# r-barnes/richdem

Measured on NVIDIA H100. Metric: Priority-Flood fill + D8 flow accumulation throughput, higher is better.
Workload: dtype f32

## Files before the change

richdem_b200/csrc/accum.cu:

```cuda
#include "flowmet.cuh"

#include <cmath>
#include <cooperative_groups.h>
namespace cg = cooperative_groups;

namespace rdb {

namespace {

constexpr uint32_t kDepsMask = 0xFFu;
constexpr uint32_t kSrcFlag = 0x80000000u;
constexpr int kCodeSole = 32;
constexpr int kCodeSource = 64;
constexpr int kLaneChunk = 1024;

template <bool DINF>
__global__ void __launch_bounds__(256) flow_code_kernel(const float *__restrict__ dem, uint8_t *__restrict__ code,
                                                         float *__restrict__ rmaxArr, double *__restrict__ accum,
                                                         int W, int H, float nodata, int ones, int tfilter) {
  const size_t n = (size_t)W * H;
  const size_t i = (size_t)blockIdx.x * blockDim.x + threadIdx.x;
  if (i >= n) return;
  const int y = (int)(i / W), x = (int)(i - (size_t)y * W);
  int cd;
// ... 1292 lines not shown
                      DinfShare *share, unsigned long long *stats, int ghost_lo_end, int ghost_hi_start, int seeded) {
  Ctx &c = ctx();
  int per_sm = 0;
  if (stats) RDB_CK(cudaOccupancyMaxActiveBlocksPerMultiprocessor(&per_sm, accum_walk_dinf_lanes_kernel<true>, 256, 0));
  else RDB_CK(cudaOccupancyMaxActiveBlocksPerMultiprocessor(&per_sm, accum_walk_dinf_lanes_kernel<false>, 256, 0));
  if (per_sm < 1) per_sm = 1;
  long long nb = (long long)c.num_sms * per_sm;
  const long long work = seeded >= 0 ? ((long long)seeded + 31) / 32 : ((long long)ncells + kLaneChunk - 1) / kLaneChunk;
  if (nb * 8 > work) nb = (work + 7) / 8;
  if (seeded >= 0 && nb < c.num_sms) nb = c.num_sms;
  if (nb < 1) nb = 1;
  if (seeded >= 0) {
    dinf_share_seed_kernel<<<1, 1, 0, c.stream>>>(share, seeded, (int)nb * 8, ncells);
    RDB_CK(cudaGetLastError());
  }
  const uint8_t *a_code = code;
  const float *a_rmax = rmax;
  int a_w = W, a_n = ncells;
  int *a_list = list;
  unsigned a_cap = (unsigned)ncells;
  DinfShare *a_sh = share;
  int a_excess = (int)(c.params.accum_dinf_share >= 0 ? c.params.accum_dinf_share : 1);
  int a_wait = (int)(c.params.accum_dinf_wait > 0 ? c.params.accum_dinf_wait : 4);
  if (a_excess > kLaneQueueD - 96) a_excess = kLaneQueueD - 96;
  unsigned long long *a_stats = stats;
  int a_lo = ghost_lo_end, a_hi = ghost_hi_start, a_seeded = seeded >= 0 ? 1 : 0;
  void *args[] = {(void *)&a_code, (void *)&a_rmax, (void *)&word, (void *)&a_w, (void *)&a_n, (void *)&a_list, (void *)&a_cap,
                  (void *)&a_sh, (void *)&a_excess, (void *)&a_wait, (void *)&a_stats, (void *)&a_lo, (void *)&a_hi, (void *)&a_seeded};
  if (stats)
    RDB_CK(cudaLaunchCooperativeKernel((const void *)accum_walk_dinf_lanes_kernel<true>, dim3((unsigned)nb), dim3(256), args, 0, c.stream));
  else
    RDB_CK(cudaLaunchCooperativeKernel((const void *)accum_walk_dinf_lanes_kernel<false>, dim3((unsigned)nb), dim3(256), args, 0, c.stream));
  RDB_CK(cudaGetLastError());
}

template <bool BAND>
void launch_walk_packed(const uint8_t *code, unsigned long long *word, int W, int ncells, const int *frontier,
                        int ghost_lo_end, int ghost_hi_start, bool src_in_code, int *cursor_buf = nullptr) {
  Ctx &c = ctx();
  if (ncells <= 0) return;
  if (c.params.accum_walk_lanes) {
    DevBuf<int> cursor;
    if (!cursor_buf) cursor.alloc(1);
    int *cur = cursor_buf ? cursor_buf : cursor.p;
    RDB_CK(cudaMemsetAsync(cur, 0, sizeof(int), c.stream));
    int per_sm = 0;
    RDB_CK(cudaOccupancyMaxActiveBlocksPerMultiprocessor(&per_sm, accum_walk_packed_lanes_kernel<BAND>, 256, 0));
    if (per_sm < 1) per_sm = 1;
    long long blocks = (long long)c.num_sms * per_sm;
    const long long need = ((long long)ncells + kLaneChunk - 1) / kLaneChunk;
    if (blocks * 8 > need) blocks = (need + 7) / 8;
    const int in_code = src_in_code && c.params.accum_walk_scan && (ncells & 3) == 0 && ((uintptr_t)code & 3) == 0 ? (int)c.params.accum_walk_scan : 0;
    int ahead = (int)(c.params.accum_walk_ahead > 0 ? c.params.accum_walk_ahead : 64);
    if (ahead > kLaneQueue - 128) ahead = kLaneQueue - 128;
    if (ahead < 32) ahead = 32;
    accum_walk_packed_lanes_kernel<BAND><<<(unsigned)blocks, 256, 0, c.stream>>>(code, word, W, ncells, frontier, ghost_lo_end,
                                                                               ghost_hi_start, cur, in_code, ahead);
    RDB_CK(cudaGetLastError());
    if (!cursor_buf) RDB_CK(cudaStreamSynchronize(c.stream));
  } else {
    accum_walk_packed_kernel<BAND><<<(unsigned)((ncells + 255) / 256), 256, 0, c.stream>>>(code, word, W, ncells, frontier,
                                                                                        ghost_lo_end, ghost_hi_start);
  }
}

__global__ void __launch_bounds__(256) band_take_packed_kernel(unsigned long long *ghost, double *sum, int *cnt, int W,
                                                                int *total) {
  const int x = blockIdx.x * blockDim.x + threadIdx.x;
  int k = 0;
  if (x < W) {
    const unsigned long long wv = ghost[x];
    k = (int)(wv >> 56);
    sum[x] = (double)(wv & kPkVal);
    cnt[x] = k;
    ghost[x] = 0;
  }
  for (int o = 16; o > 0; o >>= 1) k += __shfl_down_sync(0xffffffffu, k, o);
  if ((threadIdx.x & 31) == 0 && k) atomicAdd(total, k);
}

__global__ void __launch_bounds__(256) band_count_packed_kernel(const unsigned long long *__restrict__ gtop,
                                                                 const unsigned long long *__restrict__ gbot, int W,
                                                                 int *sums) {
  int s0 = 0, s1 = 0;
  for (int x = blockIdx.x * blockDim.x + threadIdx.x; x < W; x += gridDim.x * blockDim.x) {
    if (gtop) s0 += (int)(gtop[x] >> 56);
    if (gbot) s1 += (int)(gbot[x] >> 56);
  }
  for (int o = 16; o > 0; o >>= 1) {
    s0 += __shfl_down_sync(0xffffffffu, s0, o);
    s1 += __shfl_down_sync(0xffffffffu, s1, o);
  }
  if ((threadIdx.x & 31) == 0) {
    if (s0) atomicAdd(&sums[0], s0);
    if (s1) atomicAdd(&sums[1], s1);
  }
}

__global__ void __launch_bounds__(256) band_apply_packed_kernel(unsigned long long *row, const double *__restrict__ sum,
                                                                 const int *__restrict__ cnt, int W, int base_index,
                                                                 int *frontier, int *fcount, double scale) {
  const int x = blockIdx.x * blockDim.x + threadIdx.x;
  if (x >= W) return;
  const int k = cnt[x];
  if (k <= 0) return;
  const unsigned long long wv = row[x];
  const unsigned long long val = (wv & kPkVal) + (unsigned long long)sum[x];
  const unsigned long long left = (wv >> 56) - (unsigned long long)k;
  if (left == 0) {
    row[x] = (unsigned long long)__double_as_longlong((double)val * scale);
    frontier[atomicAdd(fcount, 1)] = base_index + x;
  } else {
    row[x] = (left << 56) | val;
  }
}

constexpr int kFaT = 64;
constexpr int kFaCells = kFaT * kFaT;
constexpr int kFaSlots = 4 * kFaT;
constexpr unsigned long long kLkOne = 1ull << 32;

__device__ __forceinline__ int fa_side(int left) { return left < kFaT ? left : kFaT; }

__device__ __forceinline__ int fa_slot_of(int lx, int ly, int tw, int th) {
  if (ly == 0) return lx;
  if (ly == th - 1) return kFaT + lx;
  if (lx == 0) return 2 * kFaT + ly;
  if (lx == tw - 1) return 3 * kFaT + ly;
  return -1;
}

__device__ __forceinline__ bool fa_slot_cell(int s, int tw, int th, int &lx, int &ly) {
  const int k = s & (kFaT - 1), side = s / kFaT;
  if (side < 2) {
    lx = k;
    ly = side == 0 ? 0 : th - 1;
    return k < tw && (side == 0 || th > 1);
  }
  lx = side == 2 ? 0 : tw - 1;
  ly = k;
  return k > 0 && k < th - 1 && (side == 2 || tw > 1);
}

constexpr int kFaRootExit = 0x8000, kFaRootEnd = 0x4000, kFaRoot = kFaRootExit | kFaRootEnd;

__device__ __forceinline__ int fa_tile_parent(int c, int cd, int tw, int th) {
  const int d = cd & 15;
  if (cd == kCodeNoData || d == 0) return c | kFaRootEnd;
  const int x = (c & (kFaT - 1)) + d8dx(d), y = c / kFaT + d8dy(d);
  if (x < 0 || y < 0 || x >= tw || y >= th) return c | kFaRootExit;
  return y * kFaT + x;
}

template <bool SUM>
__device__ __forceinline__ void fa_tile_jump(uint16_t *sPar, unsigned *sAcc, unsigned live) {
  constexpr int kPer = kFaCells / 256;
  const int t = threadIdx.x;
  while (__syncthreads_or(live)) {
    unsigned pq[kPer], a[kPer];
#pragma unroll
    for (int k = 0; k < kPer; k++) {
      if (live >> k & 1) {
        const int c = t + 256 * k, p = sPar[c], q = sPar[p];
        if (SUM) {
          pq[k] = (unsigned)p | (unsigned)q << 16;
          a[k] = sAcc[c];
        } else {
          sPar[c] = (uint16_t)q;
          if (q & kFaRoot) live &= ~(1u << k);
        }
      }
    }
    if (SUM) {
      __syncthreads();
#pragma unroll
      for (int k = 0; k < kPer; k++) {
        if (live >> k & 1) {
          const int q = pq[k] >> 16;
          atomicAdd(&sAcc[pq[k] & 0xffffu], a[k]);
          sPar[t + 256 * k] = (uint16_t)q;
          if (q & kFaRoot) live &= ~(1u << k);
        }
      }
    }
  }
}

__global__ void __launch_bounds__(256) fa_tile_codes_kernel(const float *__restrict__ dem, uint8_t *__restrict__ code,
                                                             int *__restrict__ link, unsigned long long *__restrict__ lword,
                                                             unsigned *__restrict__ inflow, int W, int H, float nodata,
                                                             int tiles_x) {
  constexpr int kWin = kFaT + 2;
  static_assert(kFaCells * sizeof(uint16_t) <= kWin * kWin * sizeof(float), "the parent array lives in the DEM window");
  __shared__ __align__(16) float sDem[kWin * kWin];
  __shared__ __align__(16) uint8_t sCode[kFaCells];
  __shared__ unsigned sCount[kFaSlots];
  const int t = threadIdx.x, tile = blockIdx.x;
  sCount[t] = 0;
  const int bx = tile % tiles_x, by = tile / tiles_x;
  const int x0 = bx * kFaT, y0 = by * kFaT;
  const int tw = fa_side(W - x0), th = fa_side(H - y0);
  constexpr unsigned kFaNoDataBits = 0x7fffffffu;
  for (int i = t; i < kWin * kWin; i += 256) {
    const int wy = i / kWin, wx = i - wy * kWin;
    const int gy = y0 - 1 + wy, gx = x0 - 1 + wx;
    float v = __uint_as_float(kFaNoDataBits);
    if (gy >= 0 && gy < H && gx >= 0 && gx < W) {
      v = __ldg(dem + (size_t)gy * W + gx);
      v = v == nodata ? __uint_as_float(kFaNoDataBits) : v != v ? __uint_as_float(0x7fc00000u) : v;
    }
    sDem[i] = v;
  }
  __syncthreads();
  {
    const int lx0 = (t & 15) * 4, ly0 = (t >> 4) * 4;
    float a[3][6];
#pragma unroll
    for (int j = 1; j < 3; j++)
#pragma unroll
      for (int k = 0; k < 6; k++) a[j][k] = sDem[(ly0 + j - 1) * kWin + lx0 + k];
#pragma unroll
    for (int j = 0; j < 4; j++) {
      const int ly = ly0 + j, gy = y0 + ly;
#pragma unroll
      for (int k = 0; k < 6; k++) {
        a[0][k] = a[1][k];
        a[1][k] = a[2][k];
        a[2][k] = sDem[(ly + 2) * kWin + lx0 + k];
      }
      unsigned word = 0;
#pragma unroll
      for (int k = 0; k < 4; k++) {
        const int lx = lx0 + k, gx = x0 + lx;
        const float e = a[1][k + 1];
        int cd = 0;
        if (lx >= tw || ly >= th || __float_as_uint(e) == kFaNoDataBits) {
          cd = kCodeNoData;
        } else if (!(gx == 0 || gy == 0 || gx == W - 1 || gy == H - 1)) {
          const float ne[9] = {0.f, a[1][k], a[0][k], a[0][k + 1], a[0][k + 2], a[1][k + 2], a[2][k + 2], a[2][k + 1], a[2][k]};
          float lowest = fminf(e, 3.402823466e+38f);
#pragma unroll
          for (int n = 1; n <= 8; n++) {
            if (ne[n] < lowest) {
              lowest = ne[n];
              cd = n;
            }
          }
        }
        word |= (unsigned)cd << (8 * k);
      }
      *reinterpret_cast<unsigned *>(&sCode[ly * kFaT + lx0]) = word;
    }
  }
  __syncthreads();
  reinterpret_cast<uint4 *>(code + (size_t)tile * kFaCells)[t] = reinterpret_cast<const uint4 *>(sCode)[t];
  uint16_t *sPar = reinterpret_cast<uint16_t *>(sDem);
  unsigned live = 0;
#pragma unroll
  for (int k = 0; k < kFaCells / 256; k++) {
    const int c = t + 256 * k, p = fa_tile_parent(c, sCode[c], tw, th);
    sPar[c] = (uint16_t)p;
    if (!(p & kFaRoot)) live |= 1u << k;
  }
  fa_tile_jump<false>(sPar, nullptr, live);
#pragma unroll
  for (int k = 0; k < kFaCells / 256; k++) {
    const int r = sPar[t + 256 * k];
    if (r & kFaRootExit) atomicAdd(&sCount[fa_slot_of(r & (kFaT - 1), (r & (kFaCells - 1)) / kFaT, tw, th)], 1u);
  }
  __syncthreads();
  const size_t gs = (size_t)tile * kFaSlots + t;
  int lk = -1;
  unsigned long long out = 0;
  int lx, ly;
  if (fa_slot_cell(t, tw, th, lx, ly)) {
    const int c = ly * kFaT + lx, r = sPar[c];
    if (r == (c | kFaRootExit)) {
      const int d = sCode[c] & 15;
      const int gx = x0 + lx + d8dx(d), gy = y0 + ly + d8dy(d), rbx = gx / kFaT, rby = gy / kFaT;
      const int rs = fa_slot_of(gx - rbx * kFaT, gy - rby * kFaT, fa_side(W - rbx * kFaT), fa_side(H - rby * kFaT));
      lk = -2 - ((rby * tiles_x + rbx) * kFaSlots + rs);
      out = kLkOne | sCount[t];
    } else if (r & kFaRootExit) {
      const int e = r & (kFaCells - 1);
      lk = tile * kFaSlots + fa_slot_of(e & (kFaT - 1), e / kFaT, tw, th);
    }
  }
  link[gs] = lk;
  lword[gs] = out;
  inflow[gs] = 0;
}

__device__ __forceinline__ int fa_link_next(const int *link, int r) {
  const int l = link[r];
  return l <= -2 ? r : l;
}

__global__ void __launch_bounds__(256) fa_link_count_kernel(const int *__restrict__ link, unsigned long long *lword,
                                                             int nslots) {
  const int p = blockIdx.x * blockDim.x + threadIdx.x;
  if (p >= nslots) return;
  const int l = link[p];
  if (l > -2) return;
  const int q = fa_link_next(link, -2 - l);
  if (q >= 0) atomicAdd(&lword[q], kLkOne);
}

__global__ void __launch_bounds__(256) fa_link_walk_kernel(const int *__restrict__ link, unsigned long long *lword,
                                                            unsigned *inflow, int nslots) {
  const int p = blockIdx.x * blockDim.x + threadIdx.x;
  if (p >= nslots) return;
  int l = link[p];
  if (l > -2) return;
  const unsigned long long old = atomicAdd(&lword[p], 0ull - kLkOne);
  if ((old >> 32) != 1ull) return;
  unsigned long long acc = old & (kLkOne - 1);
  for (;;) {
    const int r = -2 - l;
    atomicAdd(&inflow[r], (unsigned)acc);
    const int q = fa_link_next(link, r);
    if (q < 0) break;
    const unsigned long long o = atomicAdd(&lword[q], acc - kLkOne);
    if ((o >> 32) != 1ull) break;
    acc = (o & (kLkOne - 1)) + acc;
    l = link[q];
  }
}

__global__ void __launch_bounds__(256) fa_tile_final_kernel(const uint8_t *__restrict__ code,
                                                             const unsigned *__restrict__ inflow, double *__restrict__ accum,
                                                             int W, int H, int tiles_x) {
  constexpr unsigned kNoDataAcc = 0xffffffffu;
  __shared__ __align__(16) unsigned sAcc[kFaCells];
  __shared__ __align__(16) uint16_t sPar[kFaCells];
  __shared__ __align__(16) uint8_t sCode[kFaCells];
  const int t = threadIdx.x, tile = blockIdx.x;
  const int bx = tile % tiles_x, by = tile / tiles_x;
  const int x0 = bx * kFaT, y0 = by * kFaT;
  const int tw = fa_side(W - x0), th = fa_side(H - y0);
  reinterpret_cast<uint4 *>(sCode)[t] = __ldg(reinterpret_cast<const uint4 *>(code + (size_t)tile * kFaCells) + t);
  __syncthreads();
  unsigned live = 0;
#pragma unroll
  for (int k = 0; k < kFaCells / 256; k++) {
    const int c = t + 256 * k, cd = sCode[c], p = fa_tile_parent(c, cd, tw, th);
    sPar[c] = (uint16_t)p;
    sAcc[c] = cd == kCodeNoData ? kNoDataAcc : 1u;
    if (!(p & kFaRoot)) live |= 1u << k;
  }
  __syncthreads();
  int lx, ly;
  if (fa_slot_cell(t, tw, th, lx, ly) && sCode[ly * kFaT + lx] != kCodeNoData)
    sAcc[ly * kFaT + lx] += __ldg(inflow + (size_t)tile * kFaSlots + t);
  fa_tile_jump<true>(sPar, sAcc, live);
  for (int c = 2 * t; c < kFaCells; c += 512) {
    const int cx = c & (kFaT - 1), cy = c / kFaT;
    if (cx >= tw || cy >= th) continue;
    const unsigned s0 = sAcc[c], s1 = sAcc[c + 1];
    const double a0 = s0 == kNoDataAcc ? -1.0 : (double)s0, a1 = s1 == kNoDataAcc ? -1.0 : (double)s1;
    double *out = accum + (size_t)(y0 + cy) * W + x0 + cx;
    if (cx + 1 < tw && ((uintptr_t)out & 15) == 0) {
      *reinterpret_cast<double2 *>(out) = make_double2(a0, a1);
    } else {
      out[0] = a0;
      if (cx + 1 < tw) out[1] = a1;
    }
  }
}

long long fa_tile_slots(int w, int h) {
  return (long long)((w + kFaT - 1) / kFaT) * ((h + kFaT - 1) / kFaT) * kFaSlots;
}

void fa_d8_tiles(const float *d_dem, double *d_accum, int w, int h, float nodata) {
  Ctx &c = ctx();
  const int tiles_x = (w + kFaT - 1) / kFaT;
  const long long nslots = fa_tile_slots(w, h);
  const unsigned ntiles = (unsigned)(nslots / kFaSlots);
  DevBuf<uint8_t> code((size_t)ntiles * kFaCells);
  DevBuf<int> link((size_t)nslots);
  DevBuf<unsigned long long> lword((size_t)nslots);
  DevBuf<unsigned> inflow((size_t)nslots);
  const unsigned sblocks = (unsigned)((nslots + 255) / 256);
  fa_tile_codes_kernel<<<ntiles, 256, 0, c.stream>>>(d_dem, code.p, link.p, lword.p, inflow.p, w, h, nodata, tiles_x);
  fa_link_count_kernel<<<sblocks, 256, 0, c.stream>>>(link.p, lword.p, (int)nslots);
  KernelTimer kt;
  fa_link_walk_kernel<<<sblocks, 256, 0, c.stream>>>(link.p, lword.p, inflow.p, (int)nslots);
  kt.stop_async();
  fa_tile_final_kernel<<<ntiles, 256, 0, c.stream>>>(code.p, inflow.p, d_accum, w, h, tiles_x);
  RDB_CK(cudaGetLastError());
  count_launch(4);
  RDB_CK(cudaStreamSynchronize(c.stream));
  c.stats.ms_main_kernel += kt.ms();
  c.stats.accum_rounds = 1;
}
}

void fa_fused_dev(const float *d_dem, double *d_accum, int w, int h, float nodata, bool ones, bool dinf) {
  Ctx &c = ctx();
  const size_t n = (size_t)w * h;
  if (!dinf && ones && c.params.accum_packed && fa_tile_slots(w, h) < INT32_MAX) {
    fa_d8_tiles(d_dem, d_accum, w, h, nodata);
    return;
  }
  DevBuf<uint8_t> code(n);
  DevBuf<float> rmax;
  bool have_codes = false;
  if (dinf && ones && (w & 3) == 0 && ((uintptr_t)d_accum & 15) == 0 && c.params.accum_dinf_packed) {
    rmax.alloc(n);
    const unsigned blocks = (unsigned)((n + 255) / 256);
    unsigned long long *word = reinterpret_cast<unsigned long long *>(d_accum);
    flow_code_kernel<true><<<blocks, 256, 0, c.stream>>>(d_dem, code.p, rmax.p, d_accum, w, h, nodata, 1, (int)c.params.flowmet_tarboton_filter);
    have_codes = true;
    DevBuf<DinfShare> share(1);
    RDB_CK(cudaMemsetAsync(share.p, 0, sizeof(DinfShare), c.stream));
    dinf_count_data_kernel<<<c.num_sms * 8, 256, 0, c.stream>>>(code.p, n, share.p);
    RDB_CK(cudaGetLastError());
    count_launch(2);
    DinfShare *hs0 = reinterpret_cast<DinfShare *>(c.pinned);
    RDB_CK(cudaMemcpyAsync(hs0, share.p, sizeof(DinfShare), cudaMemcpyDeviceToHost, c.stream));
    RDB_CK(cudaStreamSynchronize(c.stream));
    const bool use_packed = c.params.accum_dinf_packed == 1 || (long long)hs0->n_noflow * 20 > (long long)hs0->n_data;
    if (use_packed) {
    dim3 blk(256), grd((w / 4 + 255) / 256, h < 8192 ? h : 8192);
    deps_gather_packed_dinf_x4_kernel<<<grd, blk, 0, c.stream>>>(code.p, word, w, h, 0, h);
    RDB_CK(cudaGetLastError());
    count_launch();
    DevBuf<int> list(n);
    DevBuf<unsigned long long> dstats;
    if (c.params.accum_dinf_stats) {
      dstats.alloc(16);
      RDB_CK(cudaMemsetAsync(dstats.p, 0, 16 * sizeof(unsigned long long), c.stream));
    }
    KernelTimer kt;
    launch_walk_dinf(code.p, rmax.p, word, w, (int)n, list.p, share.p, dstats.p, 0, (int)n, -1);
    RDB_CK(cudaGetLastError());
    count_launch(2);
    DinfShare *hs = reinterpret_cast<DinfShare *>(c.pinned);
    RDB_CK(cudaMemcpyAsync(hs, share.p, sizeof(DinfShare), cudaMemcpyDeviceToHost, c.stream));
    kt.stop_async();
    RDB_CK(cudaStreamSynchronize(c.stream));
    c.stats.ms_main_kernel += kt.ms();
    c.stats.accum_rounds = hs->phases;
    if (dstats.p) {
      unsigned long long hsx[16];
      RDB_CK(cudaMemcpy(hsx, dstats.p, sizeof(hsx), cudaMemcpyDeviceToHost));
      fprintf(stderr,
              "[dinf walk] %.2f ms, %llu warps, %d phases: iterations sum %llu max %llu, lane-steps %llu (%.1f %% of the lanes), "
              "hand-overs %llu in the rings, %llu through the list (%llu claimed back)\n",
              kt.ms(), hsx[4], hs->phases, hsx[0], hsx[3], hsx[2], 100.0 * (double)hsx[2] / (32.0 * (double)(hsx[0] ? hsx[0] : 1)),
              hsx[8], hsx[7], hsx[6]);
    }
    if (hs->done != hs->n_data)
      fail("D-infinity accumulation (packed walk): %d of %d cells walked after %d phases", hs->done, hs->n_data, hs->phases);
    return;
    }
  }
  DevBuf<uint32_t> st(n);
  if (dinf && !have_codes) rmax.alloc(n);
  const unsigned blocks = (unsigned)((n + 255) / 256);
  if (have_codes) {
  } else if (dinf)
    flow_code_kernel<true><<<blocks, 256, 0, c.stream>>>(d_dem, code.p, rmax.p, d_accum, w, h, nodata, ones ? 1 : 0, (int)c.params.flowmet_tarboton_filter);
  else if ((w & 3) == 0 && ((uintptr_t)d_dem & 15) == 0 && ((uintptr_t)d_accum & 15) == 0) {
    dim3 blk(256), grd((w / 4 + 255) / 256, h < 8192 ? h : 8192);
    flow_code_d8_x4_kernel<<<grd, blk, 0, c.stream>>>(d_dem, code.p, d_accum, w, h, nodata, ones ? 1 : 0);
  } else
    flow_code_kernel<false><<<blocks, 256, 0, c.stream>>>(d_dem, code.p, nullptr, d_accum, w, h, nodata, ones ? 1 : 0, (int)c.params.flowmet_tarboton_filter);
  RDB_CK(cudaGetLastError());
  if ((w & 3) == 0) {
    dim3 blk(256), grd((w / 4 + 255) / 256, h < 8192 ? h : 8192);
    deps_gather_x4_kernel<<<grd, blk, 0, c.stream>>>(code.p, st.p, w, h, 0, h, dinf ? 0 : 1);
  } else {
    deps_gather_kernel<<<blocks, 256, 0, c.stream>>>(code.p, st.p, w, h, 0, h, dinf ? 0 : 1);
  }
  RDB_CK(cudaGetLastError());
  count_launch(2);
  WalkArgs<double> a;
  memset(&a, 0, sizeof(a));
  a.code = code.p;
  a.rmaxArr = rmax.p;
  a.accum = d_accum;
  a.st = st.p;
  a.W = w;
  a.H = h;
  if (dinf) run_levels<1>(a, n);
  else run_walk<0, false, double>(a, n);
}

void flow_accumulation_props_dev(const float *d_props, double *d_accum, int w, int h) {
  Ctx &c = ctx();
  const size_t n = (size_t)w * h;
  DevBuf<uint32_t> st(n);
  RDB_CK(cudaMemsetAsync(st.p, 0, n * sizeof(uint32_t), c.stream));
  const unsigned blocks = (unsigned)((n + 255) / 256);
  deps_scatter_props_kernel<<<blocks, 256, 0, c.stream>>>(d_props, st.p, w, h);
  RDB_CK(cudaGetLastError());
  mark_sources_props_kernel<<<blocks, 256, 0, c.stream>>>(d_props, st.p, d_accum, n);
  RDB_CK(cudaGetLastError());
  count_launch(2);
  WalkArgs<double> a;
  memset(&a, 0, sizeof(a));
  a.props = d_props;
  a.accum = d_accum;
  a.st = st.p;
  a.W = w;
  a.H = h;
  run_levels<2>(a, n);
}

void d8_flow_accum_dev(const uint8_t *d_dirs, int32_t *d_area, int w, int h) {
  Ctx &c = ctx();
  const size_t n = (size_t)w * h;
  DevBuf<uint8_t> code(n);
  DevBuf<uint32_t> st(n);
  const unsigned blocks = (unsigned)((n + 255) / 256);
  sanitize_dirs_kernel<<<blocks, 256, 0, c.stream>>>(d_dirs, code.p, n);
  area_init_kernel<<<blocks, 256, 0, c.stream>>>(d_dirs, d_area, n);
  deps_gather_kernel<<<blocks, 256, 0, c.stream>>>(code.p, st.p, w, h, 0, h, 1);
  RDB_CK(cudaGetLastError());
  count_launch(3);
  WalkArgs<int32_t> a;
  memset(&a, 0, sizeof(a));
  a.code = code.p;
  a.accum = d_area;
  a.st = st.p;
  a.W = w;
  a.H = h;
  run_walk<0, true, int32_t>(a, n);
  area_unreleased_kernel<<<blocks, 256, 0, c.stream>>>(st.p, d_area, n);
  RDB_CK(cudaGetLastError());
  count_launch();
}

}

namespace rdb {
namespace {

__global__ void __launch_bounds__(256) band_apply_inflow_kernel(double *accum_row, uint32_t *st_row,
                                                                 const double *__restrict__ sum,
                                                                 const int *__restrict__ cnt, int W, int base_index,
                                                                 int *frontier, int *fcount) {
  const int x = blockIdx.x * blockDim.x + threadIdx.x;
  if (x >= W) return;
  const int k = cnt[x];
  if (k <= 0) return;
// ... 753 lines not shown
```

richdem_b200/csrc/capi.cu:

```cuda
#include "common.cuh"

#include <algorithm>
#include <cstdlib>

namespace rdb {

static thread_local std::string g_last_error;

void capi_set_error(const char *msg) { g_last_error = msg ? msg : "unknown error"; }

Ctx &ctx() {
  static Ctx c;
  return c;
}

static void init_device(int device) {
  Ctx &c = ctx();
  if (c.inited && c.device == device) return;
  if (c.inited) fail("rdb200_init: already initialised on device %d (call rdb200_shutdown first)", c.device);
  int ndev = 0;
  cudaError_t e = cudaGetDeviceCount(&ndev);
  if (e != cudaSuccess || ndev == 0)
    fail("no CUDA device available (%s); librichdem_b200 has no CPU fallback",
         e == cudaSuccess ? "device count is 0" : cudaGetErrorString(e));
// ... 75 lines not shown
      it = c.ws.erase(it);
    } else {
      ++it;
    }
  }
}

void ws_release_all() {
  Ctx &c = ctx();
  for (auto &b : c.ws) cudaFree(b.ptr);
  c.ws.clear();
}

struct CallScope {
  explicit CallScope(int64_t cells) {
    ensure_init();
    Ctx &c = ctx();
    memset(&c.stats, 0, sizeof(c.stats));
    c.stats.cells = cells;
    RDB_CK(cudaEventRecord(c.ev0, c.stream));
  }
  void done() {
    Ctx &c = ctx();
    RDB_CK(cudaEventRecord(c.ev1, c.stream));
    RDB_CK(cudaStreamSynchronize(c.stream));
    float ms = 0;
    RDB_CK(cudaEventElapsedTime(&ms, c.ev0, c.ev1));
    c.stats.ms_total = ms;
  }
};

static void check_dims(int w, int h) {
  if (w <= 0 || h <= 0) fail("raster dimensions must be positive (got %d x %d)", w, h);
  if ((int64_t)w * h > ((int64_t)1 << 31) - ((int64_t)1 << 25))
    fail("rasters above 2^31 - 2^25 cells per GPU are not supported (got %d x %d); shard by rows", w, h);
}

template <class T>
static void h2d(T *dst, const T *src, size_t n) {
  Ctx &c = ctx();
  cudaEvent_t a = c.evk0, b = c.evk1;
  RDB_CK(cudaEventRecord(a, c.stream));
  RDB_CK(cudaMemcpyAsync(dst, src, n * sizeof(T), cudaMemcpyHostToDevice, c.stream));
  RDB_CK(cudaEventRecord(b, c.stream));
  RDB_CK(cudaStreamSynchronize(c.stream));
  float ms = 0;
  RDB_CK(cudaEventElapsedTime(&ms, a, b));
  c.stats.ms_h2d += ms;
}
template <class T>
static void d2h(T *dst, const T *src, size_t n) {
  Ctx &c = ctx();
  cudaEvent_t a = c.evk0, b = c.evk1;
  RDB_CK(cudaEventRecord(a, c.stream));
  RDB_CK(cudaMemcpyAsync(dst, src, n * sizeof(T), cudaMemcpyDeviceToHost, c.stream));
  RDB_CK(cudaEventRecord(b, c.stream));
  RDB_CK(cudaStreamSynchronize(c.stream));
  float ms = 0;
  RDB_CK(cudaEventElapsedTime(&ms, a, b));
  c.stats.ms_d2h += ms;
}

}

using namespace rdb;

#define CAPI_TRY try {
#define CAPI_END                    \
  }                                 \
  catch (const std::exception &e) { \
    capi_set_error(e.what());       \
    return 1;                       \
  }                                 \
  catch (...) {                     \
    capi_set_error("unknown C++ exception"); \
    return 1;                       \
  }                                 \
  return 0;

extern "C" {

int rdb200_init(int device) {
  CAPI_TRY
  init_device(device);
  CAPI_END
}

void rdb200_shutdown(void) {
  Ctx &c = ctx();
  if (!c.inited) return;
  cudaSetDevice(c.device);
  cudaStreamSynchronize(c.stream);
  ws_release_all();
  if (c.pinned) cudaFreeHost(c.pinned);
  cudaEventDestroy(c.ev0);
  cudaEventDestroy(c.ev1);
  cudaEventDestroy(c.evk0);
  cudaEventDestroy(c.evk1);
  cudaStreamDestroy(c.own_stream);
  for (int k = 0; k < 2; k++)
    if (c.aux_stream[k]) cudaStreamDestroy(c.aux_stream[k]);
  for (int k = 0; k < 3; k++)
    if (c.aux_event[k]) cudaEventDestroy(c.aux_event[k]);
  const Params keep = c.params;
  c = Ctx();
  c.params = keep;
}

const char *rdb200_last_error(void) { return g_last_error.c_str(); }
int rdb200_version(void) { return RDB200_VERSION; }

int rdb200_set_stream(void *cuda_stream) {
  CAPI_TRY
  ensure_init();
  Ctx &c = ctx();
  RDB_CK(cudaStreamSynchronize(c.stream));
  c.stream = cuda_stream ? (cudaStream_t)cuda_stream : c.own_stream;
  CAPI_END
}

int rdb200_get_stats(rdb200_stats *out) {
  CAPI_TRY
  if (!out) fail("rdb200_get_stats: null pointer");
  *out = ctx().stats;
  CAPI_END
}

int rdb200_set_param(const char *name, int64_t value) {
  CAPI_TRY
  if (!name) fail("rdb200_set_param: null name");
  Params &p = ctx().params;
  const std::string n(name);
  if (n == "reset_defaults") p = Params();
  else if (n == "trim_workspace") {
    if (ctx().inited) {
      RDB_CK(cudaStreamSynchronize(ctx().stream));
      ws_trim();
    }
  }
  else if (n == "fill_max_iters") p.fill_max_iters = value;
  else if (n == "fill_rounds_per_sync") p.fill_rounds_per_sync = value > 0 ? value : 16;
  else if (n == "fill_use_tma") p.fill_use_tma = value;
  else if (n == "fill_external_z") p.fill_external_z = value;
  else if (n == "fill_profile") p.fill_profile = value;
  else if (n == "fill_wake_filter") p.fill_wake_filter = value;
  else if (n == "fill_trace") p.fill_trace = value;
  else if (n == "fill_ordered") p.fill_ordered = value;
  else if (n == "fill_order_rounds") p.fill_order_rounds = value;
  else if (n == "fill_band_rounds") p.fill_band_rounds = value;
  else if (n == "accum_threads") p.accum_threads = value > 0 ? value : 256;
  else if (n == "accum_budget") p.accum_budget = value;
  else if (n == "accum_walk_lanes") p.accum_walk_lanes = value;
  else if (n == "accum_fused_prep") p.accum_fused_prep = value;
  else if (n == "flats_tiled") p.flats_tiled = value;
  else if (n == "flats_pair") p.flats_pair = value;
  else if (n == "flats_fused_classify") p.flats_fused_classify = value;
  else if (n == "fill_multigrid") p.fill_multigrid = value;
  else if (n == "fill_multigrid_min") p.fill_multigrid_min = value;
  else if (n == "fill_vcycle") p.fill_vcycle = value;
  else if (n == "fill_band_multigrid") p.fill_band_multigrid = value;
  else if (n == "flats_uf_tiled") p.flats_uf_tiled = value;
  else if (n == "flowdirs_rolling") p.flowdirs_rolling = value;
  else if (n == "accum_packed") p.accum_packed = value;
  else if (n == "accum_dinf_packed") p.accum_dinf_packed = value;
  else if (n == "accum_dinf_share") p.accum_dinf_share = value;
  else if (n == "flowmet_tarboton_filter") p.flowmet_tarboton_filter = value;
  else if (n == "accum_walk_scan") p.accum_walk_scan = value;
  else if (n == "accum_walk_ahead") p.accum_walk_ahead = value;
  else if (n == "accum_dinf_stats") p.accum_dinf_stats = value;
  else if (n == "accum_dinf_wait") p.accum_dinf_wait = value;
  else fail("rdb200_set_param: unknown parameter '%s'", name);
  CAPI_END
}


int rdb200_fill_depressions_d8_f32(float *dem, int32_t w, int32_t h) {
  CAPI_TRY
  if (!dem) fail("fill_depressions: null dem");
  check_dims(w, h);
  CallScope cs((int64_t)w * h);
  const size_t n = (size_t)w * h;
  DevBuf<float> d(n);
  h2d(d.p, dem, n);
  fill_depressions_dev(d.p, w, h);
  d2h(dem, d.p, n);
  cs.done();
  CAPI_END
}

int rdb200_fill_depressions_d4_f32(float *dem, int32_t w, int32_t h) {
  CAPI_TRY
  if (!dem) fail("fill_depressions: null dem");
  check_dims(w, h);
  CallScope cs((int64_t)w * h);
  const size_t n = (size_t)w * h;
  DevBuf<float> d(n);
  h2d(d.p, dem, n);
  fill_depressions_dev(d.p, w, h, true);
  d2h(dem, d.p, n);
  cs.done();
  CAPI_END
}

static int pit_mask_host(const float *dem, uint8_t *mask, int32_t w, int32_t h, float nodata, bool topo4) {
  CAPI_TRY
  if (!dem || !mask) fail("pit_mask: null pointer");
  check_dims(w, h);
  CallScope cs((int64_t)w * h);
  const size_t n = (size_t)w * h;
  DevBuf<float> d(n);
  DevBuf<uint8_t> m(n);
  h2d(d.p, dem, n);
  pit_mask_dev(d.p, m.p, w, h, nodata, topo4);
  d2h(mask, m.p, n);
  cs.done();
  CAPI_END
}
int rdb200_pit_mask_d8_f32(const float *dem, uint8_t *mask, int32_t w, int32_t h, float nodata) {
  return pit_mask_host(dem, mask, w, h, nodata, false);
}
int rdb200_pit_mask_d4_f32(const float *dem, uint8_t *mask, int32_t w, int32_t h, float nodata) {
  return pit_mask_host(dem, mask, w, h, nodata, true);
}

static int has_depressions_host(const float *dem, int32_t w, int32_t h, int32_t *out, bool topo4) {
  CAPI_TRY
  if (!dem || !out) fail("has_depressions: null pointer");
  check_dims(w, h);
  CallScope cs((int64_t)w * h);
  const size_t n = (size_t)w * h;
  DevBuf<float> d(n);
  h2d(d.p, dem, n);
  const bool any = has_depressions_dev(d.p, w, h, topo4);
  cs.done();
  *out = any ? 1 : 0;
  CAPI_END
}
int rdb200_has_depressions_d8_f32(const float *dem, int32_t w, int32_t h, int32_t *out) {
  return has_depressions_host(dem, w, h, out, false);
}
int rdb200_has_depressions_d4_f32(const float *dem, int32_t w, int32_t h, int32_t *out) {
  return has_depressions_host(dem, w, h, out, true);
}

int rdb200_resolve_flats_epsilon_f32(float *dem, int32_t w, int32_t h, float nodata) {
  CAPI_TRY
  if (!dem) fail("resolve_flats: null dem");
  check_dims(w, h);
  CallScope cs((int64_t)w * h);
  const size_t n = (size_t)w * h;
  DevBuf<float> d(n);
  h2d(d.p, dem, n);
  resolve_flats_dev(d.p, w, h, nodata, nullptr, nullptr, true);
  d2h(dem, d.p, n);
  cs.done();
  CAPI_END
}

int rdb200_get_flat_mask_f32(const float *dem, int32_t *flat_mask, int32_t *labels, int32_t w, int32_t h,
                             float nodata) {
  CAPI_TRY
  if (!dem || !flat_mask || !labels) fail("get_flat_mask: null pointer");
  check_dims(w, h);
  CallScope cs((int64_t)w * h);
  const size_t n = (size_t)w * h;
  DevBuf<float> d(n);
  DevBuf<int32_t> m(n), l(n);
  h2d(d.p, dem, n);
  resolve_flats_dev(d.p, w, h, nodata, m.p, l.p, false);
  d2h(flat_mask, m.p, n);
  d2h(labels, l.p, n);
  cs.done();
  CAPI_END
}

int rdb200_d8_flow_directions_f32(const float *dem, uint8_t *dirs, int32_t w, int32_t h, float nodata) {
  CAPI_TRY
  if (!dem || !dirs) fail("d8_flow_directions: null pointer");
  check_dims(w, h);
  CallScope cs((int64_t)w * h);
  const size_t n = (size_t)w * h;
  DevBuf<float> d(n);
  DevBuf<uint8_t> o(n);
  h2d(d.p, dem, n);
  d8_flow_directions_dev(d.p, o.p, w, h, nodata);
  d2h(dirs, o.p, n);
  cs.done();
  CAPI_END
}

int rdb200_d8_flow_directions_flats_f32(float *dem, uint8_t *dirs, int32_t w, int32_t h, float nodata, int32_t alter) {
  CAPI_TRY
  if (!dem || !dirs) fail("d8_flow_directions_flats: null pointer");
  check_dims(w, h);
  CallScope cs((int64_t)w * h);
  const size_t n = (size_t)w * h;
  DevBuf<float> d(n);
  DevBuf<uint8_t> o(n);
  h2d(d.p, dem, n);
  d8_flow_directions_flats_dev(d.p, o.p, w, h, nodata, alter != 0);
  d2h(dirs, o.p, n);
  if (alter) d2h(dem, d.p, n);
  cs.done();
  CAPI_END
}

// ... 629 lines not shown
```

richdem_b200/csrc/common.cuh:

```cuda
#pragma once

#include <cuda.h>
#include <cuda_runtime.h>

#include <cstdarg>
#include <cstdint>
#include <cstdio>
#include <cstring>
#include <stdexcept>
#include <string>
#include <vector>

#include "../../include/richdem_b200.h"

struct rdb200_fill_state;

namespace rdb {

struct Error : std::runtime_error {
  using std::runtime_error::runtime_error;
};

[[noreturn]] inline void fail(const char *fmt, ...) {
  char buf[1024];
  va_list ap;
  va_start(ap, fmt);
  vsnprintf(buf, sizeof(buf), fmt, ap);
  va_end(ap);
  throw Error(buf);
}

#define RDB_CK(expr)                                                                        \
  do {                                                                                      \
    cudaError_t _e = (expr);                                                                \
    if (_e != cudaSuccess)                                                                  \
      ::rdb::fail("%s failed at %s:%d: %s", #expr, __FILE__, __LINE__, cudaGetErrorString(_e)); \
  } while (0)

__host__ __device__ __forceinline__ int d8dx(int n) {
  return (int)((0x6a41u >> (2 * n)) & 3u) - 1;
}
__host__ __device__ __forceinline__ int d8dy(int n) {
  return (int)((0x2a405u >> (2 * n)) & 3u) - 1;
}

struct Params {
  int64_t fill_max_iters = 0;
  int64_t fill_rounds_per_sync = 16;
  int64_t fill_use_tma = 1;
  int64_t fill_external_z = 1;
  int64_t fill_ordered = 1;
  int64_t fill_order_rounds = 0;
  int64_t fill_band_rounds = 0;
  int64_t fill_profile = 0;
  int64_t fill_wake_filter = 1;
  int64_t fill_trace = 0;
  int64_t fill_multigrid = 8;
  int64_t fill_vcycle = 8;
  int64_t fill_band_multigrid = 0;
  int64_t fill_multigrid_min = 0;
  int64_t flowdirs_rolling = 1;
  int64_t flats_uf_tiled = 1;
  int64_t flats_fused_classify = 1;
  int64_t flats_pair = 1;
  int64_t flats_tiled = 1;
  int64_t accum_dinf_packed = 1;
  int64_t flowmet_tarboton_filter = 1;
  int64_t accum_walk_ahead = 0;
  int64_t accum_walk_scan = 0;
  int64_t accum_dinf_stats = 0;
  int64_t accum_dinf_share = -1;
  int64_t accum_dinf_wait = 0;
  int64_t accum_packed = 1;
  int64_t accum_fused_prep = 1;
  int64_t accum_walk_lanes = 1;
  int64_t accum_threads = 256;
  int64_t accum_budget = 0;
};

struct WsBlock {
  void *ptr;
  size_t bytes;
  bool in_use;
};

struct Ctx {
  bool inited = false;
  int device = -1;
  int num_sms = 0;
  cudaStream_t stream = nullptr;
  cudaStream_t own_stream = nullptr;
  cudaEvent_t ev0 = nullptr, ev1 = nullptr, evk0 = nullptr, evk1 = nullptr;
  cudaStream_t aux_stream[2] = {nullptr, nullptr};
  cudaEvent_t aux_event[3] = {nullptr, nullptr, nullptr};
  std::vector<WsBlock> ws;
  void *pinned = nullptr;
  size_t pinned_bytes = 0;
  rdb200_stats stats;
  Params params;
};

Ctx &ctx();
void ensure_init();
void *ws_alloc(size_t bytes);
void ws_free(void *p);
void ws_release_all();

template <class T>
struct DevBuf {
  T *p = nullptr;
  size_t n = 0;
  DevBuf() = default;
  explicit DevBuf(size_t count) { alloc(count); }
  void alloc(size_t count) {
    reset();
    n = count;
    p = (T *)ws_alloc((count ? count : 1) * sizeof(T));
  }
  void reset() {
    if (p) ws_free(p);
    p = nullptr;
    n = 0;
  }
  ~DevBuf() { reset(); }
  DevBuf(const DevBuf &) = delete;
  DevBuf &operator=(const DevBuf &) = delete;
  operator T *() const { return p; }
};

inline void count_launch(int64_t k = 1) { ctx().stats.kernel_launches += k; }

struct KernelTimer {
  bool active;
  explicit KernelTimer(bool on = true) : active(on) {
    if (active) RDB_CK(cudaEventRecord(ctx().evk0, ctx().stream));
  }
  void stop_async() {
    if (active) RDB_CK(cudaEventRecord(ctx().evk1, ctx().stream));
  }
  double ms() {
    float t = 0;
    if (active) RDB_CK(cudaEventElapsedTime(&t, ctx().evk0, ctx().evk1));
    return t;
  }
};

int comm_rank(const rdb200_comm *c);
int comm_world(const rdb200_comm *c);
void comm_exchange(const rdb200_comm *c, const void *send_up, void *recv_up, const void *send_dn, void *recv_dn, size_t bytes);
void comm_allreduce(const rdb200_comm *c, void *buf, size_t count, int op);
void check_band_args(const char *what, const rdb200_comm *comm, const void *d_band, int w, int hloc, int gt, int gb);
void exchange_band_rows(const rdb200_comm *comm, void *d_band, size_t elem, int w, int hloc, int gt, int gb);
void mgpu_fill_band(const rdb200_comm *comm, float *d_local, int w, int hloc, int gt, int gb, int row0, int H, int *xrounds,
                    bool topo4 = false);
void mgpu_fa_band(const rdb200_comm *comm, const float *d_dem, double *d_accum, int w, int hloc, float nodata, int gt, int gb,
                  int method, double xparam, bool ones, int *xrounds);
void mgpu_flow_accumulation_props_band(const rdb200_comm *comm, float *d_props, double *d_accum, int w, int hloc, int gt, int gb,
                                       int *xrounds);
void mgpu_resolve_flats_band(const rdb200_comm *comm, float *d_local, int w, int hloc, float nodata, int gt, int gb,
                             int *seam_iters);
void mgpu_d8_flow_directions_flats_band(const rdb200_comm *comm, float *d_dem, uint8_t *d_dirs, int w, int hloc, float nodata,
                                        int gt, int gb, bool alter, int *seam_iters);
void mgpu_d8_flow_accum_band(const rdb200_comm *comm, const uint8_t *d_dirs, int32_t *d_area, int w, int hloc, int gt, int gb,
                             int *xrounds);
int mgpu_relax_band(const rdb200_comm *comm, rdb200_fill_state *state, int gt, int gb, int R);

void fill_depressions_dev(float *d_dem, int w, int h, bool topo4 = false);
void geodesic_distance_dev(const uint8_t *d_open, int open_bit, float *d_w_inout, int w, int h);
void geodesic_distance_pair_dev(const uint8_t *d_open, int open_bit, float *d_wa, float *d_wb, int w, int h);
rdb200_fill_state *new_band_distance_state(const uint8_t *d_open, int open_bit, const float *d_winit, int w, int h,
                                           int ghost_top, int ghost_bottom);
void finish_band_distance_state(rdb200_fill_state *s, float *d_out);
void resolve_flats_dev(float *d_dem, int w, int h, float nodata, int32_t *d_mask_out,
                       int32_t *d_labels_out, bool apply, const uint8_t *d_dirs = nullptr);
void d8_flow_directions_flats_dev(float *d_dem, uint8_t *d_dirs, int w, int h, float nodata, bool alter);
void d8_flow_directions_dev(const float *d_dem, uint8_t *d_dirs, int w, int h, float nodata);
void d8_flow_accum_dev(const uint8_t *d_dirs, int32_t *d_area, int w, int h);
void fm_d8_dev(const float *d_dem, float *d_props, int w, int h, float nodata);
void fm_tarboton_dev(const float *d_dem, float *d_props, int w, int h, float nodata);
void fm_d4_dev(const float *d_dem, float *d_props, int w, int h, float nodata);
void fm_holmgren_dev(const float *d_dem, float *d_props, int w, int h, float nodata, double xparam);
void fm_freeman_dev(const float *d_dem, float *d_props, int w, int h, float nodata, double xparam);
void flow_accumulation_props_dev(const float *d_props, double *d_accum, int w, int h);
void fa_fused_dev(const float *d_dem, double *d_accum, int w, int h, float nodata, bool ones,
                  bool dinf);
void terrain_attribute_dev(int attribute_id, const float *d_dem, float *d_out, int w, int h, float nodata_in, float nodata_out,
                           float zscale, double cell_x, double cell_y);
void generate_fbm_dev(float *d_dem, int w, int h, int y0, uint32_t seed, int octaves, float quantum);
void pit_mask_dev(const float *d_dem, uint8_t *d_mask, int w, int h, float nodata, bool topo4);
bool has_depressions_dev(const float *d_dem, int w, int h, bool topo4);
void mgpu_pit_mask_band(const rdb200_comm *comm, const float *d_band, uint8_t *d_mask, int w, int hloc, float nodata, int gt,
                        int gb, int row0, int H, bool topo4);
bool mgpu_has_depressions_band(const rdb200_comm *comm, const float *d_band, int w, int hloc, int gt, int gb, int row0, int H,
                               bool topo4);
void pit_mask_compare_dev(const float *d_z, const float *d_l, uint8_t *d_mask, size_t n, float nodata, int *d_any);
void strict_pit_f64_dev(const double *d_z, int w, int h, bool topo4, int *d_flag);
void d8_flow_directions_f64_dev(const double *d_dem, uint8_t *d_dirs, int w, int h, double nodata);

float f64_keys_dev(const double *d_z, float *d_key, size_t n, double nodata, DevBuf<double> *table, int *ranked);
void fill_depressions_f64_dev(double *d_z, int w, int h, bool topo4);
void pit_mask_f64_dev(const double *d_z, uint8_t *d_mask, int w, int h, double nodata, bool topo4);
bool has_depressions_f64_dev(const double *d_z, int w, int h, bool topo4);
void resolve_flats_f64_dev(double *d_z, int w, int h, double nodata);
void fa_d8_f64_dev(const double *d_z, double *d_accum, int w, int h, double nodata, bool ones);

}
```

Before: 22190.

## Vectorize tile DEM window load, reshape code stencil, add phase profiler

Replaces the scalar strided halo-window load with float4 row loads plus a separate path for the left and right halo columns. The direction-code stencil changes from 4x4 cells per thread to 2x8 cells per thread, reading rows with 64-bit shared loads. The pass-1 kernel gets launch bounds asking for 8 blocks per SM, and the final kernel loads its inflow value early. It also adds an opt-in clock64 phase profiler that is off by default, though the kernel now takes an extra pointer argument and branches on it.

```diff
diff --git a/richdem_b200/csrc/accum.cu b/richdem_b200/csrc/accum.cu
--- a/richdem_b200/csrc/accum.cu
+++ b/richdem_b200/csrc/accum.cu
@@ -1468,6 +1468,28 @@
   return y * kFaT + x;
 }
 
+enum {
+  kFaProfWindow, kFaProfCodes, kFaProfParents, kFaProfJump, kFaProfCount, kFaProfSlots,
+  kFaProfFinalInit, kFaProfFinalJump, kFaProfFinalWrite,
+  kFaProfN
+};
+
+__device__ __forceinline__ long long fa_clock() {
+  long long t = 0;
+  asm volatile("mov.u64 %0, %%clock64;" : "=l"(t));
+  return t;
+}
+
+__device__ __forceinline__ void fa_phase(unsigned long long *prof, int phase, long long &t0) {
+  if (!prof) return;
+  __syncthreads();
+  if (threadIdx.x == 0) {
+    const long long t1 = fa_clock();
+    atomicAdd(prof + phase, (unsigned long long)(t1 - t0));
+    t0 = t1;
+  }
+}
+
 template <bool SUM>
 __device__ __forceinline__ void fa_tile_jump(uint16_t *sPar, unsigned *sAcc, unsigned live) {
   constexpr int kPer = kFaCells / 256;
@@ -1502,51 +1524,84 @@
   }
 }
 
-__global__ void __launch_bounds__(256) fa_tile_codes_kernel(const float *__restrict__ dem, uint8_t *__restrict__ code,
+__global__ void __launch_bounds__(256, 8) fa_tile_codes_kernel(const float *__restrict__ dem, uint8_t *__restrict__ code,
                                                              int *__restrict__ link, unsigned long long *__restrict__ lword,
                                                              unsigned *__restrict__ inflow, int W, int H, float nodata,
-                                                             int tiles_x) {
+                                                             int tiles_x, unsigned long long *prof) {
   constexpr int kWin = kFaT + 2;
   static_assert(kFaCells * sizeof(uint16_t) <= kWin * kWin * sizeof(float), "the parent array lives in the DEM window");
   __shared__ __align__(16) float sDem[kWin * kWin];
   __shared__ __align__(16) uint8_t sCode[kFaCells];
   __shared__ unsigned sCount[kFaSlots];
   const int t = threadIdx.x, tile = blockIdx.x;
+  long long clk = prof ? fa_clock() : 0;
   sCount[t] = 0;
   const int bx = tile % tiles_x, by = tile / tiles_x;
   const int x0 = bx * kFaT, y0 = by * kFaT;
   const int tw = fa_side(W - x0), th = fa_side(H - y0);
   constexpr unsigned kFaNoDataBits = 0x7fffffffu;
-  for (int i = t; i < kWin * kWin; i += 256) {
-    const int wy = i / kWin, wx = i - wy * kWin;
-    const int gy = y0 - 1 + wy, gx = x0 - 1 + wx;
-    float v = __uint_as_float(kFaNoDataBits);
-    if (gy >= 0 && gy < H && gx >= 0 && gx < W) {
-      v = __ldg(dem + (size_t)gy * W + gx);
-      v = v == nodata ? __uint_as_float(kFaNoDataBits) : v != v ? __uint_as_float(0x7fc00000u) : v;
-    }
-    sDem[i] = v;
+  const float kNd = __uint_as_float(kFaNoDataBits);
+  auto canon = [&](float v) { return v == nodata ? kNd : v != v ? __uint_as_float(0x7fc00000u) : v; };
+  {
+    const int h = t & 15;
+    const bool vec = (W & 3) == 0 && ((uintptr_t)dem & 15) == 0;
+    float4 v[5];
+#pragma unroll
+    for (int i = 0; i < 5; i++) {
+      const int wy = (t >> 4) + 16 * i, gy = y0 - 1 + wy;
+      v[i] = make_float4(kNd, kNd, kNd, kNd);
+      if (wy < kWin && gy >= 0 && gy < H) {
+        const float *src = dem + (size_t)gy * W + x0 + 4 * h;
+        if (vec) {
+          if (4 * h < tw) v[i] = __ldg(reinterpret_cast<const float4 *>(src));
+        } else {
+          if (4 * h < tw) v[i].x = __ldg(src);
+          if (4 * h + 1 < tw) v[i].y = __ldg(src + 1);
+          if (4 * h + 2 < tw) v[i].z = __ldg(src + 2);
+          if (4 * h + 3 < tw) v[i].w = __ldg(src + 3);
+        }
+      }
+    }
+    const int j = t - 32, awy = j >> 1, ax = j & 1 ? tw : -1, agy = y0 - 1 + awy;
+    float ap = kNd;
+    if (j >= 0 && j < 2 * kWin && agy >= 0 && agy < H && x0 + ax >= 0 && x0 + ax < W)
+      ap = __ldg(dem + (size_t)agy * W + x0 + ax);
+#pragma unroll
+    for (int i = 0; i < 5; i++) {
+      const int wy = (t >> 4) + 16 * i;
+      if (wy < kWin) {
+        float *cell = sDem + wy * kWin + 1 + 4 * h;
+        cell[0] = canon(v[i].x), cell[1] = canon(v[i].y), cell[2] = canon(v[i].z), cell[3] = canon(v[i].w);
+      }
+    }
+    if (j >= 0 && j < 2 * kWin) sDem[awy * kWin + (j & 1 ? tw + 1 : 0)] = canon(ap);
   }
   __syncthreads();
+  fa_phase(prof, kFaProfWindow, clk);
   {
-    const int lx0 = (t & 15) * 4, ly0 = (t >> 4) * 4;
-    float a[3][6];
-#pragma unroll
-    for (int j = 1; j < 3; j++)
-#pragma unroll
-      for (int k = 0; k < 6; k++) a[j][k] = sDem[(ly0 + j - 1) * kWin + lx0 + k];
-#pragma unroll
-    for (int j = 0; j < 4; j++) {
+    constexpr int CW = 2, RH = 8;
+    const int lx0 = (t & 31) * 2, ly0 = (t >> 5) * 8;
+    float a[3][CW + 2];
+    auto load_row = [&](float(&dst)[CW + 2], int wy) {
+      const unsigned long long *src = reinterpret_cast<const unsigned long long *>(sDem + wy * kWin + lx0);
+      const unsigned long long p = src[0], q = src[1];
+      dst[0] = __uint_as_float((unsigned)p), dst[1] = __uint_as_float((unsigned)(p >> 32));
+      dst[2] = __uint_as_float((unsigned)q), dst[3] = __uint_as_float((unsigned)(q >> 32));
+    };
+    load_row(a[1], ly0);
+    load_row(a[2], ly0 + 1);
+#pragma unroll
+    for (int j = 0; j < RH; j++) {
       const int ly = ly0 + j, gy = y0 + ly;
 #pragma unroll
-      for (int k = 0; k < 6; k++) {
+      for (int k = 0; k < CW + 2; k++) {
         a[0][k] = a[1][k];
         a[1][k] = a[2][k];
-        a[2][k] = sDem[(ly + 2) * kWin + lx0 + k];
-      }
+      }
+      load_row(a[2], ly + 2);
       unsigned word = 0;
 #pragma unroll
-      for (int k = 0; k < 4; k++) {
+      for (int k = 0; k < CW; k++) {
         const int lx = lx0 + k, gx = x0 + lx;
         const float e = a[1][k + 1];
         int cd = 0;
@@ -1565,10 +1620,11 @@
         }
         word |= (unsigned)cd << (8 * k);
       }
-      *reinterpret_cast<unsigned *>(&sCode[ly * kFaT + lx0]) = word;
+      *reinterpret_cast<uint16_t *>(&sCode[ly * kFaT + lx0]) = (uint16_t)word;
     }
   }
   __syncthreads();
+  fa_phase(prof, kFaProfCodes, clk);
   reinterpret_cast<uint4 *>(code + (size_t)tile * kFaCells)[t] = reinterpret_cast<const uint4 *>(sCode)[t];
   uint16_t *sPar = reinterpret_cast<uint16_t *>(sDem);
   unsigned live = 0;
@@ -1578,13 +1634,16 @@
     sPar[c] = (uint16_t)p;
     if (!(p & kFaRoot)) live |= 1u << k;
   }
+  fa_phase(prof, kFaProfParents, clk);
   fa_tile_jump<false>(sPar, nullptr, live);
+  fa_phase(prof, kFaProfJump, clk);
 #pragma unroll
   for (int k = 0; k < kFaCells / 256; k++) {
     const int r = sPar[t + 256 * k];
     if (r & kFaRootExit) atomicAdd(&sCount[fa_slot_of(r & (kFaT - 1), (r & (kFaCells - 1)) / kFaT, tw, th)], 1u);
   }
   __syncthreads();
+  fa_phase(prof, kFaProfCount, clk);
   const size_t gs = (size_t)tile * kFaSlots + t;
   int lk = -1;
   unsigned long long out = 0;
@@ -1605,6 +1664,7 @@
   link[gs] = lk;
   lword[gs] = out;
   inflow[gs] = 0;
+  fa_phase(prof, kFaProfSlots, clk);
 }
 
 __device__ __forceinline__ int fa_link_next(const int *link, int r) {
@@ -1645,15 +1705,17 @@
 
 __global__ void __launch_bounds__(256) fa_tile_final_kernel(const uint8_t *__restrict__ code,
                                                              const unsigned *__restrict__ inflow, double *__restrict__ accum,
-                                                             int W, int H, int tiles_x) {
+                                                             int W, int H, int tiles_x, unsigned long long *prof) {
   constexpr unsigned kNoDataAcc = 0xffffffffu;
   __shared__ __align__(16) unsigned sAcc[kFaCells];
   __shared__ __align__(16) uint16_t sPar[kFaCells];
   __shared__ __align__(16) uint8_t sCode[kFaCells];
   const int t = threadIdx.x, tile = blockIdx.x;
+  long long clk = prof ? fa_clock() : 0;
   const int bx = tile % tiles_x, by = tile / tiles_x;
   const int x0 = bx * kFaT, y0 = by * kFaT;
   const int tw = fa_side(W - x0), th = fa_side(H - y0);
+  const unsigned in = __ldg(inflow + (size_t)tile * kFaSlots + t);
   reinterpret_cast<uint4 *>(sCode)[t] = __ldg(reinterpret_cast<const uint4 *>(code + (size_t)tile * kFaCells) + t);
   __syncthreads();
   unsigned live = 0;
@@ -1667,8 +1729,10 @@
   __syncthreads();
   int lx, ly;
   if (fa_slot_cell(t, tw, th, lx, ly) && sCode[ly * kFaT + lx] != kCodeNoData)
-    sAcc[ly * kFaT + lx] += __ldg(inflow + (size_t)tile * kFaSlots + t);
+    sAcc[ly * kFaT + lx] += in;
+  fa_phase(prof, kFaProfFinalInit, clk);
   fa_tile_jump<true>(sPar, sAcc, live);
+  fa_phase(prof, kFaProfFinalJump, clk);
   for (int c = 2 * t; c < kFaCells; c += 512) {
     const int cx = c & (kFaT - 1), cy = c / kFaT;
     if (cx >= tw || cy >= th) continue;
@@ -1682,6 +1746,7 @@
       if (cx + 1 < tw) out[1] = a1;
     }
   }
+  fa_phase(prof, kFaProfFinalWrite, clk);
 }
 
 long long fa_tile_slots(int w, int h) {
@@ -1697,18 +1762,32 @@
   DevBuf<int> link((size_t)nslots);
   DevBuf<unsigned long long> lword((size_t)nslots);
   DevBuf<unsigned> inflow((size_t)nslots);
+  DevBuf<unsigned long long> prof;
+  if (c.params.fa_profile) {
+    prof.alloc(kFaProfN);
+    RDB_CK(cudaMemsetAsync(prof.p, 0, kFaProfN * sizeof(unsigned long long), c.stream));
+  }
   const unsigned sblocks = (unsigned)((nslots + 255) / 256);
-  fa_tile_codes_kernel<<<ntiles, 256, 0, c.stream>>>(d_dem, code.p, link.p, lword.p, inflow.p, w, h, nodata, tiles_x);
+  fa_tile_codes_kernel<<<ntiles, 256, 0, c.stream>>>(d_dem, code.p, link.p, lword.p, inflow.p, w, h, nodata, tiles_x, prof.p);
   fa_link_count_kernel<<<sblocks, 256, 0, c.stream>>>(link.p, lword.p, (int)nslots);
   KernelTimer kt;
   fa_link_walk_kernel<<<sblocks, 256, 0, c.stream>>>(link.p, lword.p, inflow.p, (int)nslots);
   kt.stop_async();
-  fa_tile_final_kernel<<<ntiles, 256, 0, c.stream>>>(code.p, inflow.p, d_accum, w, h, tiles_x);
+  fa_tile_final_kernel<<<ntiles, 256, 0, c.stream>>>(code.p, inflow.p, d_accum, w, h, tiles_x, prof.p);
   RDB_CK(cudaGetLastError());
   count_launch(4);
   RDB_CK(cudaStreamSynchronize(c.stream));
   c.stats.ms_main_kernel += kt.ms();
   c.stats.accum_rounds = 1;
+  if (prof.p) {
+    unsigned long long hp[kFaProfN];
+    RDB_CK(cudaMemcpy(hp, prof.p, sizeof(hp), cudaMemcpyDeviceToHost));
+    const double nt = ntiles;
+    fprintf(stderr, "[fa_d8 profile] tiles=%u pass1_cycles_per_tile window=%.0f codes=%.0f parents=%.0f jump=%.0f count=%.0f "
+            "records=%.0f pass3_cycles_per_tile init=%.0f jump=%.0f write=%.0f\n", ntiles, hp[kFaProfWindow] / nt, hp[kFaProfCodes] / nt,
+            hp[kFaProfParents] / nt, hp[kFaProfJump] / nt, hp[kFaProfCount] / nt, hp[kFaProfSlots] / nt,
+            hp[kFaProfFinalInit] / nt, hp[kFaProfFinalJump] / nt, hp[kFaProfFinalWrite] / nt);
+  }
 }
 }
 
diff --git a/richdem_b200/csrc/capi.cu b/richdem_b200/csrc/capi.cu
--- a/richdem_b200/csrc/capi.cu
+++ b/richdem_b200/csrc/capi.cu
@@ -251,6 +251,7 @@
   else if (n == "accum_budget") p.accum_budget = value;
   else if (n == "accum_walk_lanes") p.accum_walk_lanes = value;
   else if (n == "accum_fused_prep") p.accum_fused_prep = value;
+  else if (n == "fa_profile") p.fa_profile = value;
   else if (n == "flats_tiled") p.flats_tiled = value;
   else if (n == "flats_pair") p.flats_pair = value;
   else if (n == "flats_fused_classify") p.flats_fused_classify = value;
diff --git a/richdem_b200/csrc/common.cuh b/richdem_b200/csrc/common.cuh
--- a/richdem_b200/csrc/common.cuh
+++ b/richdem_b200/csrc/common.cuh
@@ -72,6 +72,7 @@
   int64_t accum_dinf_share = -1;
   int64_t accum_dinf_wait = 0;
   int64_t accum_packed = 1;
+  int64_t fa_profile = 0;
   int64_t accum_fused_prep = 1;
   int64_t accum_walk_lanes = 1;
   int64_t accum_threads = 256;
```

Result: faster. 22610 (median of 6 runs) (+1.9%).
